# hendraet/synthesis-in-style

Hardware: AMD Instinct MI355X
Metric: StyleGAN2 synth images/sec + seg-train images/sec @256², 1/2/4/8 MI355X (higher is better)
Workload: dtype f32; 1 GPU; StyleGAN2 Generator(256,512,8,cm=2).forward, batch 32 per GPU, explicit noise, return_intermediate_activations=True (BASELINE.json configs[1]); batch_per_gpu=32, image_size=256, parallelism=replicated x1, images sharded, no collective

## Files before the change

### include/sis_hip.h

```cpp
#ifndef SIS_HIP_H
#define SIS_HIP_H

#include <stdint.h>

#ifdef __cplusplus
extern "C" {
#endif

#define SIS_F32 0
#define SIS_F64 1
#define SIS_F16 2
#define SIS_BF16 3

int sis_version(void);
const char* sis_last_error(void);
const char* sis_last_kernel(void);

int sis_fused_bias_act(void* out, const void* x, const void* bias, const void* ref, int dtype,
                       int64_t numel, int64_t step_b, int64_t size_b, int act, int grad,
                       float alpha, float scale, void* stream);

int sis_upfirdn2d_out_size(int in_size, int up, int down, int pad0, int pad1, int k);
int sis_upfirdn2d(void* out, const void* in, const void* taps, int dtype, int major, int in_h,
                  int in_w, int minor, int kh, int kw, int up_x, int up_y, int down_x, int down_y,
                  int pad_x0, int pad_x1, int pad_y0, int pad_y1, void* stream);


int sis_pixel_norm(float* out, const float* x, int batch, int dim, void* stream);

int sis_head_gemm_tile(void);

int sis_equal_linear(float* out, const float* x, int64_t x_row_stride, const float* w,
                     const float* bias, int batch, int in_dim, int out_dim, float scale,
                     float lr_mul, int activation, void* stream);

int sis_modulation_batch(float* out_base, const float* latent, const int64_t* table, int n_layers,
                         int total_blocks, int batch, int n_latent, int dim, float scale, void* stream);

int sis_demod_batch(float* dscale_base, const float* s_base, const int64_t* table, int n_layers,
                    int total_blocks, int batch, void* stream);

int sis_truncate(float* out, const float* w, const float* mean, float psi, int batch, int dim,
                 void* stream);

int sis_modconv_prepack(float* wpk, float* wsq, const float* w, int cout, int cin, int ksize,
                        void* stream);

int sis_modconv_demod(float* dscale, const float* s, const float* wsq, int batch, int cin,
                      int cout, float scale, int demodulate, void* stream);

int sis_modconv2d(float* out, const float* x, const float* wpk, const float* s,
                  const float* dscale, const float* noise, int64_t noise_batch_stride,
                  const float* noise_weight, const float* bias, int batch, int cin, int cout,
                  int h, int w, int ksize, int fuse_act, const float* wino_u, void* workspace,
                  int64_t workspace_bytes, void* stream);

int sis_modconv_prepack_wino(float* u, const float* w, int cout, int cin, void* stream);

int sis_modconv2d_up(float* t, const float* x, const float* wpk, const float* s,
                     const float* dscale, int batch, int cin, int cout, int h, int w,
                     int t_row_stride, void* workspace, int64_t workspace_bytes, void* stream);

int sis_modconv_up_fir_supported(int batch, int cin, int cout, int h, int w, int t_row_stride);
int sis_modconv_up_fir_prepack(float* u, const float* w, int cout, int cin, void* stream);
int sis_modconv2d_up_fir(float* t, const float* x, const float* u, const float* s, const float* dscale, int batch, int cin, int cout,
                         int h, int w, int t_row_stride, void* stream);

int sis_blur_noise_act(float* out, const float* in, const float* taps, const float* noise,
                       int64_t noise_batch_stride, const float* noise_weight, const float* bias,
                       int batch, int channels, int in_h, int in_w, int in_row_stride, int kh, int kw,
                       int pad0, int pad1, int fuse_act, void* stream);

int sis_to_rgb(float* out, const float* x, const float* w, const float* s, const float* bias,
               const float* skip, const float* taps, int batch, int cin, int cout, int h, int width,
               int kh, int kw, int pad0, int pad1, float scale, void* stream);


int sis_upsample_ce_workspace(int batch, int out_h, int out_w);
int sis_upsample_ce_fwd(float* loss, float* workspace, const float* logits, const int64_t* labels,
                        int batch, int classes, int h, int w, int out_h, int out_w,
                        int64_t ignore_index, void* stream);
int sis_upsample_ce_bwd(float* grad_logits, const float* grad_loss, const float* logits,
                        const int64_t* labels, int batch, int classes, int h, int w, int out_h,
                        int out_w, int64_t ignore_index, void* stream);

int sis_sgd_chunk_elems(void);
int sis_sgd_momentum(const int64_t* table, int n_chunks, const float* lr, const float* weight_decay,
                     int n_groups, float momentum, int first_step, void* stream);

int sis_sgd_momentum_dev(const int64_t* table, int n_chunks, const float* hyper, void* stream);

int sis_ema_update(float* mu, const float* mu_batch, float momentum, float one_minus_momentum,
                   int batch, int numel, void* stream);

int sis_half_dilation_taps(float* taps, const float* weight, int cout, int cin, void* stream);
int sis_half_dilation_taps_bwd(float* dweight, const float* dtaps, int cout, int cin, void* stream);

int sis_emau_supported(int batch, int channels, int pixels, int bases);
int64_t sis_emau_workspace_floats(int batch, int channels, int pixels, int bases);
int sis_emau_forward(float* x_out, float* mu_out, const float* x, const float* mu0, float* workspace, int batch, int channels,
                     int pixels, int bases, int stages, void* stream);

int64_t sis_bn_workspace_floats(int batch, int channels, int hw);
int64_t sis_bn_mask_words(int batch, int channels, int hw);
int sis_bn_stats(float* mean, float* invstd, float* running_mean, float* running_var, const float* x,
                 float* workspace, int batch, int channels, int hw, float eps, float momentum, void* stream);
int sis_bn_act_fwd(float* y, const float* x, const float* residual, const float* mean, const float* invstd,
                   const float* gamma, const float* beta, int batch, int channels, int hw, int relu, void* relu_mask,
                   void* stream);
int sis_bn_act_bwd(float* dx, float* dresidual, float* dgamma, float* dbeta, const float* dy, const float* y,
// ... 237 lines not shown
```

### synthesis-in-style_amd/csrc/modconv_wino.hip

```cpp
#include "modconv_common.h"

#if !defined(SIS_ABLATIONS) && (defined(SIS_WINO_NODMA) || defined(SIS_WINO_NOTRANSFORM) || defined(SIS_WINO_NOBARRIER) || \
                                defined(SIS_WINO_NOSTORE) || defined(SIS_WINO_STAGGER))
#error "SIS_WINO_* ablation switches need -DSIS_ABLATIONS (development builds only)"
#endif

namespace {

constexpr int WCC = 8;
#ifndef SIS_WINO_BAR_SLOT
#define SIS_WINO_BAR_SLOT 27
#endif
constexpr int S_BAR = SIS_WINO_BAR_SLOT;
constexpr int WMBLK = 64;
constexpr int WTILES = 64;

__device__ __forceinline__ sis_f32x4 lds_ld4(const float* p) { return *reinterpret_cast<const sis_f32x4*>(p); }
__device__ __forceinline__ void lds_st4(float* p, sis_f32x2 a, sis_f32x2 b) { *reinterpret_cast<sis_f32x4*>(p) = sis_f32x4{a.x, a.y, b.x, b.y}; }
__device__ __forceinline__ float2 lds_ld2(const float* p) {
    const sis_f32x2 d = *reinterpret_cast<const sis_f32x2*>(p);
    return make_float2(d.x, d.y);
}
constexpr unsigned BUF_OOB = 0x80000000u;
__device__ __forceinline__ sis_f32x2 pk_lo_np_plus(sis_f32x2 y, sis_f32x2 np, sis_f32x2 x) {
// ... 834 lines not shown
        const int64_t out_bytes = (int64_t)p.B * p.Cout * p.OH * p.ORS * 4;
        if ((int64_t)want * out_bytes > workspace_bytes) want = (int)(workspace_bytes / out_bytes);
        if (want >= 2) {
            p.kchunk = sis_cdiv(sis_cdiv(p.Cin, want), WCC) * WCC;
            p.ksplit = sis_cdiv(p.Cin, p.kchunk);
            p.slab = (float*)workspace;
        }
    }
    const size_t lds = (size_t)(2 * WCC * 16 * WMBLK + 2 * WCC * tc.xt + (p.s ? p.nb_max * p.Cin : 0)) * sizeof(float);
    const size_t lds2 = lds + (size_t)(2 * 16 * WCC * WTILES + p.nb_max * WMBLK + WMBLK + WTILES * 4) * sizeof(float);
    if (lds > 160 * 1024) return -1;
    if (plan_only) return 0;
    static bool attr_set = false;
    if (!attr_set) {
        hipError_t e = hipFuncSetAttribute(reinterpret_cast<const void*>(&modconv_wino_kernel),
                                           hipFuncAttributeMaxDynamicSharedMemorySize, 160 * 1024);
        if (e != hipSuccess) return sis_fail("modconv: cannot raise the dynamic LDS limit: %s", hipGetErrorString(e));
        attr_set = true;
    }
    static const bool pipelined = !(getenv("SIS_WINO_PIPE") && getenv("SIS_WINO_PIPE")[0] == '0');
    if (pipelined && lds2 <= 160 * 1024 && tc.xt >= 256) {
        sis_kernel_name = "modconv_wino2_kernel";
        static const int tpw_cap = getenv("SIS_WINO_TPW") ? atoi(getenv("SIS_WINO_TPW")) : 16;
        int tpw = 1;
        static const int min_wg = getenv("SIS_WINO_MINWG") ? atoi(getenv("SIS_WINO_MINWG")) : 1024;
        while (p.kchunk % (2 * WCC) == 0 && tpw * 2 <= tpw_cap && p.npos_tiles % (tpw * 2) == 0 && blocks / (tpw * 2) >= min_wg) tpw *= 2;
        static const double swz_mb = getenv("SIS_WINO_XCD_MB") ? atof(getenv("SIS_WINO_XCD_MB")) : 5.0;
        const int64_t grid = blocks / tpw;
        const int n_co_h = (p.Cout + WMBLK - 1) / WMBLK;
        const int xcd_group = (double)p.Cin * p.Cout * 16 * sizeof(float) <= swz_mb * 1048576.0 && n_co_h > 1 && grid % (8 * n_co_h) == 0;
        typedef void (*kern_t)(const ConvParams, const int, const int, const int);
        static const kern_t table[4][2] = {{modconv_wino2_kernel<1, false>, modconv_wino2_kernel<1, true>},
                                           {modconv_wino2_kernel<2, false>, modconv_wino2_kernel<2, true>},
                                           {modconv_wino2_kernel<4, false>, modconv_wino2_kernel<4, true>},
                                           {modconv_wino2_kernel<8, false>, modconv_wino2_kernel<8, true>}};
        static bool table_attr[4][2] = {};
        const int xi_log2 = tc.xt <= 256 ? 0 : tc.xt <= 512 ? 1 : tc.xt <= 1024 ? 2 : 3;
        const kern_t kern = table[xi_log2][p.s ? 1 : 0];
        bool& have_attr = table_attr[xi_log2][p.s ? 1 : 0];
        if (!have_attr) {
            const hipError_t e = hipFuncSetAttribute(reinterpret_cast<const void*>(kern), hipFuncAttributeMaxDynamicSharedMemorySize, 160 * 1024);
            if (e != hipSuccess) return sis_fail("modconv: cannot raise the dynamic LDS limit: %s", hipGetErrorString(e));
            have_attr = true;
        }
        hipLaunchKernelGGL(kern, dim3((unsigned)grid, p.ksplit), dim3(WNTHR), lds2, st, p, tc.xt, tpw, xcd_group);
    } else {
        sis_kernel_name = "modconv_wino_kernel";
        hipLaunchKernelGGL(modconv_wino_kernel, dim3((unsigned)blocks, p.ksplit), dim3(WNTHR), lds, st, p, tc.xt);
    }
    SIS_CHECK_LAUNCH("modconv_wino_kernel");
    if (p.ksplit > 1) modconv_splitk_finish_launch(p, st);
    return 0;
}
```

### synthesis-in-style_amd/networks/stylegan2/model.py

```python
import math
import os
import random
import struct
import typing

import torch
from torch import nn
from torch.nn import functional as F

import sis_hip
from networks import hip_conv
from .op import FusedLeakyReLU, fused_leaky_relu, upfirdn2d

_NOISE_ONE_LAUNCH = os.environ.get('SIS_NOISE_ONE_LAUNCH', '1') != '0'
_RGB_STREAMS = {}


def _needs_grad(*tensors):
    return torch.is_grad_enabled() and any(t is not None and t.requires_grad for t in tensors)


def make_kernel(k):
    taps = torch.tensor(k, dtype=torch.float32)
    if taps.ndim == 1:
# ... 47 lines not shown
    def forward(self, input):
        if _needs_grad(input, self.weight, self.bias) or input.dim() != 2:
            bias = None if self.bias is None else self.bias * self.lr_mul
            if self.activation:
                return fused_leaky_relu(F.linear(input, self.weight * self.scale), bias)
            return F.linear(input, self.weight * self.scale, bias=bias)
        if input.is_contiguous():
            return sis_hip.equal_linear(input, self.weight, self.bias, self.scale, self.lr_mul, self.activation)
        if input.stride(1) != 1:
            input = input.contiguous()
            return sis_hip.equal_linear(input, self.weight, self.bias, self.scale, self.lr_mul, self.activation)
        return sis_hip.equal_linear(input, self.weight, self.bias, self.scale, self.lr_mul, self.activation,
                                    row_stride=input.stride(0), batch=input.shape[0])

    def __repr__(self):
        return f'{self.__class__.__name__}({self.weight.shape[1]}, {self.weight.shape[0]})'


class ModulatedConv2d(nn.Module):
    def __init__(self, in_channel, out_channel, kernel_size, style_dim, demodulate=True, upsample=False,
                 downsample=False, blur_kernel=[1, 3, 3, 1]):
        super().__init__()
        self.eps = 1e-8
        self.kernel_size = kernel_size
        self.in_channel = in_channel
        self.out_channel = out_channel
        self.upsample = upsample
        self.downsample = downsample
        self.demodulate = demodulate
        if upsample:
            factor = 2
            p = (len(blur_kernel) - factor) - (kernel_size - 1)
            self.blur = Blur(blur_kernel, pad=((p + 1) // 2 + factor - 1, p // 2 + 1), upsample_factor=factor)
        if downsample:
            factor = 2
            p = (len(blur_kernel) - factor) + (kernel_size - 1)
            self.blur = Blur(blur_kernel, pad=((p + 1) // 2, p // 2))
        self.scale = 1 / math.sqrt(in_channel * kernel_size ** 2)
        self.padding = kernel_size // 2
        self.weight = nn.Parameter(torch.randn(1, out_channel, in_channel, kernel_size, kernel_size))
        self.modulation = EqualLinear(style_dim, in_channel, bias_init=1)
        self._pack = None
        self._pack_key = None

    def __repr__(self):
        return (f'{self.__class__.__name__}({self.in_channel}, {self.out_channel}, {self.kernel_size}, '
                f'upsample={self.upsample}, downsample={self.downsample})')

    def packed_weights(self):
        w = self.weight
        key = (w.data_ptr(), w._version, w.device)
        if self._pack_key != key:
            self._pack = sis_hip.modconv_prepack(w.detach())
            self._wino = None
            if (self.kernel_size == 3 and not self.upsample and not self.downsample and self.in_channel % 8 == 0
                    and self.out_channel % 4 == 0 and os.environ.get("SIS_WINOGRAD", "1") != "0"):
                self._wino = sis_hip.modconv_prepack_wino(w.detach())
            self._fir = None
            if self.kernel_size == 3 and self.upsample and self.in_channel % 8 == 0 and self.out_channel % 64 == 0:
                self._fir = sis_hip.modconv_prepack_up_fir(w.detach())
            self._pack_key = key
        return self._pack

    def wino_weights(self):
        self.packed_weights()
        return self._wino

    def fir_weights(self):
        self.packed_weights()
        return self._fir

    def hip_supported(self):
        return (not self.downsample) and (self.kernel_size == 3 or (self.kernel_size == 1 and not self.upsample))

    def modulate(self, style):
        wpk, wsq = self.packed_weights()
        s = self.modulation(style)
        return wpk, s, sis_hip.modconv_demod(s, wsq, self.scale, self.demodulate)

    def forward(self, input, style):
        if _needs_grad(input, style, self.weight, self.modulation.weight) or not self.hip_supported():
            return self._forward_autograd(input, style)
        sis_hip.require_device(input, "input")
        wpk, s, dscale = self.modulate(style)
        if self.upsample:
            return self.blur(sis_hip.modconv2d_up(input, wpk, s, dscale))
        return sis_hip.modconv2d(input, wpk, s, dscale, self.kernel_size, wino_u=self.wino_weights())

    def _forward_autograd(self, input, style):
        if self.downsample or os.environ.get("SIS_MODCONV_GROUPED", "0") == "1":
            return self._forward_grouped(input, style)
        b, cin, h, w = input.shape
        k, cout = self.kernel_size, self.out_channel
        s = self.modulation(style)
        weight = self.weight[0]
        if self.demodulate:
            wsq = weight.pow(2).sum((2, 3))
            dcoef = self.scale * torch.rsqrt((self.scale * self.scale) * (s.pow(2) @ wsq.t()) + 1e-8)
        x = input * s.view(b, cin, 1, 1)
        if self.upsample:
            out = F.conv_transpose2d(x, weight.transpose(0, 1), stride=2)
        elif (k == 3 and x.is_cuda and x.is_contiguous() and hip_conv.gan_winograd_enabled()
              and sis_hip.conv3x3_supported(x, weight)):
            out = hip_conv.conv3x3(x, weight)
        else:
            out = F.conv2d(x, weight, padding=self.padding)
        out = out * dcoef.view(b, cout, 1, 1) if self.demodulate else out * self.scale
        return self.blur(out) if self.upsample else out

    def _forward_grouped(self, input, style):
        b, cin, h, w = input.shape
        k, cout = self.kernel_size, self.out_channel
        mod = self.modulation(style).view(b, 1, cin, 1, 1)
        wt = self.scale * self.weight * mod
        if self.demodulate:
            wt = wt * torch.rsqrt(wt.pow(2).sum([2, 3, 4], keepdim=True) + 1e-8)
        x = input.reshape(1, b * cin, h, w)
        if self.upsample:
            out = F.conv_transpose2d(x, wt.transpose(1, 2).reshape(b * cin, cout, k, k), stride=2, groups=b)
            return self.blur(out.view(b, cout, out.shape[2], out.shape[3]))
        if self.downsample:
            x = self.blur(input)
            x = x.reshape(1, b * cin, x.shape[2], x.shape[3])
            out = F.conv2d(x, wt.view(b * cout, cin, k, k), stride=2, groups=b)
        else:
            out = F.conv2d(x, wt.view(b * cout, cin, k, k), padding=self.padding, groups=b)
        return out.view(b, cout, out.shape[2], out.shape[3])


class NoiseInjection(nn.Module):
    def __init__(self):
        super().__init__()
        self.weight = nn.Parameter(torch.zeros(1))

    @staticmethod
    def fresh(image):
        b, _, h, w = image.shape
        return image.new_empty(b, 1, h, w).normal_()

    def forward(self, image, noise=None):
        if noise is None:
            noise = self.fresh(image)
        return image + self.weight * noise


class ConstantInput(nn.Module):
    def __init__(self, channel, size=4):
        super().__init__()
        self.input = nn.Parameter(torch.randn(1, channel, size, size))

    def forward(self, input):
        return self.input.repeat(input.shape[0], 1, 1, 1)


class StyledConv(nn.Module):
    def __init__(self, in_channel, out_channel, kernel_size, style_dim, upsample=False, blur_kernel=[1, 3, 3, 1],
                 demodulate=True):
        super().__init__()
        self.conv = ModulatedConv2d(in_channel, out_channel, kernel_size, style_dim, upsample=upsample,
                                    blur_kernel=blur_kernel, demodulate=demodulate)
        self.noise = NoiseInjection()
        self.activate = FusedLeakyReLU(out_channel)

    def forward(self, input, style, noise=None):
        conv, act = self.conv, self.activate
        fused_ok = (conv.hip_supported() and act.negative_slope == 0.2 and abs(act.scale - 2 ** 0.5) < 1e-12
                    and not _needs_grad(input, style, conv.weight, conv.modulation.weight, self.noise.weight, act.bias))
        if not fused_ok:
            return act(self.noise(conv(input, style), noise=noise))
        sis_hip.require_device(input, "input")
        wpk, s, dscale = conv.modulate(style)
        return self.forward_s(input, wpk, s, dscale, noise)

    def forward_s(self, input, wpk, s, dscale, noise=None, out=None):
        conv, act = self.conv, self.activate
        b, _, h, w = input.shape
        if conv.upsample:
            taps, pad = conv.blur.kernel, conv.blur.pad
            padded = tuple(taps.shape) == (4, 4) and pad[0] == 1
            t = sis_hip.modconv2d_up(input, wpk, s, dscale, padded_rows=padded, fir_u=conv.fir_weights())
            in_w = 2 * w + 1
            oh = t.shape[2] + pad[0] + pad[1] - taps.shape[0] + 1
            ow = in_w + pad[0] + pad[1] - taps.shape[1] + 1
            if noise is None:
                noise = input.new_empty(b, 1, oh, ow).normal_()
            return sis_hip.blur_noise_act(t, taps, pad, noise, self.noise.weight, act.bias, fuse_act=True, in_w=in_w)
        if noise is None:
            noise = input.new_empty(b, 1, h, w).normal_()
        return sis_hip.modconv2d(input, wpk, s, dscale, conv.kernel_size, noise, self.noise.weight, act.bias,
                                 fuse_act=True, wino_u=conv.wino_weights(), out=out)


class ToRGB(nn.Module):
    def __init__(self, in_channel, style_dim, upsample=True, blur_kernel=[1, 3, 3, 1]):
        super().__init__()
        if upsample:
            self.upsample = Upsample(blur_kernel)
        self.conv = ModulatedConv2d(in_channel, 3, 1, style_dim, demodulate=False)
        self.bias = nn.Parameter(torch.zeros(1, 3, 1, 1))

    def forward(self, input, style, skip=None):
        conv = self.conv
        if _needs_grad(input, style, skip, conv.weight, conv.modulation.weight, self.bias):
            out = conv(input, style) + self.bias
            return out if skip is None else out + self.upsample(skip)
        sis_hip.require_device(input, "input")
        return self.forward_s(input, conv.modulation(style), skip)

    def forward_s(self, input, s, skip=None, out=None):
        conv = self.conv
        if skip is None:
            return sis_hip.to_rgb(input, conv.weight, s, self.bias, conv.scale, out=out)
        up = self.upsample
        if up.factor != 2:
            return sis_hip.to_rgb(input, conv.weight, s, self.bias, conv.scale) + up(skip)
        return sis_hip.to_rgb(input, conv.weight, s, self.bias, conv.scale, skip, up.kernel, up.pad, out=out)


def truncate_styles(style, truncation, truncation_latent):
    if _needs_grad(style, truncation_latent) or not style.is_cuda or truncation_latent.numel() != style.shape[-1]:
        return truncation_latent + truncation * (style - truncation_latent)
    return sis_hip.truncate(style, truncation_latent, truncation)


def resolve_latents(generator, styles, inject_index, truncation, truncation_latent, input_is_latent, noise,
                    randomize_noise):
    if not input_is_latent:
        styles = [generator.style(s) for s in styles]
    if noise is None:
        noise = [None] * generator.num_layers if randomize_noise else [
            getattr(generator.noises, f'noise_{i}') for i in range(generator.num_layers)]
    if truncation < 1:
        styles = [truncate_styles(s, truncation, truncation_latent) for s in styles]
    n_latent = generator.n_latent
    if len(styles) < 2:
        latent = styles[0].unsqueeze(1).repeat(1, n_latent, 1) if styles[0].ndim < 3 else styles[0]
    else:
        if inject_index is None:
            inject_index = random.randint(1, n_latent - 1)
        latent = torch.cat([styles[0].unsqueeze(1).repeat(1, inject_index, 1),
                            styles[1].unsqueeze(1).repeat(1, n_latent - inject_index, 1)], 1)
    return latent, noise

# ... 232 lines not shown
```

### synthesis-in-style_amd/sis_hip/__init__.py

```python
import collections
import ctypes
import os

import torch

_HERE = os.path.dirname(os.path.abspath(__file__))
LIB_PATH = os.path.join(os.path.dirname(_HERE), "lib", os.environ.get("SIS_HIP_LIB", "libsis_hip.so"))

_lib = None

F32, F64, F16, BF16 = 0, 1, 2, 3
_DTYPE_CODE = {torch.float32: F32, torch.float64: F64, torch.float16: F16, torch.bfloat16: BF16}

_vp, _i, _i64, _f = ctypes.c_void_p, ctypes.c_int, ctypes.c_int64, ctypes.c_float
_d = ctypes.c_double

_SIGNATURES = {
    "sis_version": ([], _i),
    "sis_last_error": ([], ctypes.c_char_p),
    "sis_fused_bias_act": ([_vp, _vp, _vp, _vp, _i, _i64, _i64, _i64, _i, _i, _f, _f, _vp], _i),
    "sis_upfirdn2d_out_size": ([_i] * 6, _i),
    "sis_upfirdn2d": ([_vp, _vp, _vp] + [_i] * 15 + [_vp], _i),
    "sis_pixel_norm": ([_vp, _vp, _i, _i, _vp], _i),
    "sis_equal_linear": ([_vp, _vp, _i64, _vp, _vp, _i, _i, _i, _f, _f, _i, _vp], _i),
    "sis_truncate": ([_vp, _vp, _vp, _f, _i, _i, _vp], _i),
    "sis_modulation_batch": ([_vp, _vp, _vp, _i, _i, _i, _i, _i, _f, _vp], _i),
    "sis_demod_batch": ([_vp, _vp, _vp, _i, _i, _i, _vp], _i),
    "sis_modconv_prepack": ([_vp, _vp, _vp, _i, _i, _i, _vp], _i),
    "sis_modconv_demod": ([_vp, _vp, _vp, _i, _i, _i, _f, _i, _vp], _i),
    "sis_modconv2d": ([_vp, _vp, _vp, _vp, _vp, _vp, _i64, _vp, _vp] + [_i] * 7 + [_vp, _vp, _i64, _vp], _i),
    "sis_head_gemm_tile": ([], _i),
    "sis_modconv_prepack_wino": ([_vp, _vp, _i, _i, _vp], _i),
    "sis_last_kernel": ([], ctypes.c_char_p),
    "sis_conv3x3_prepack": ([_vp, _vp, _i, _i, _i, _vp], _i),
    "sis_conv3x3_prepack_both": ([_vp, _vp, _vp, _i, _i, _vp], _i),
    "sis_conv3x3_prepack_multi": ([_vp, _i, _i, _vp], _i),
    "sis_conv3x3_eligible": ([_i] * 5, _i),
    "sis_upsample_bilinear": ([_vp, _vp, _i, _i64, _i, _i, _i, _i, _i, _vp], _i),
    "sis_upsample_bilinear_strided": ([_vp, _vp, _i, _i, _i, _i, _i, _i, _i, _i64, _i, _vp], _i),
    "sis_gemm_bf16_workspace_bytes": ([_i, _i, _i], _i64),
    "sis_gemm_bf16": ([_vp] * 4 + [_i] * 8 + [_vp] * 3 + [_i] + [_vp] * 3 + [_i, _f, _i, _vp, _i64, _i, _vp], _i),
    "sis_gemm_bf16_wgrad_bias": ([_vp] * 4 + [_i] * 6 + [_vp, _i64, _i, _vp], _i),
    "sis_gemm_bf16_wgrad_multi_workspace_bytes": ([_i, _i, _i], _i64),
    "sis_gemm_bf16_wgrad_bias_multi": ([_vp] * 4 + [_i] * 6 + [_vp, _i64, _i, _vp], _i),
    "sis_gemm_bf16_batched": ([_vp] * 3 + [_i] * 9 + [_i64] * 3 + [_i, _vp, _i64, _i, _vp], _i),
    "sis_layer_norm_bwd_fused": ([_vp] * 9 + [_i, _i, _i, _i, _vp, _vp, _vp, _i, _f, _vp], _i),
    "sis_attention_fwd": ([_vp, _vp, _vp, _i, _i, _i, _vp], _i),
    "sis_attention_bwd": ([_vp] * 6 + [_i, _i, _i, _vp], _i),
    "sis_ce_dice_workspace_floats": ([_i], _i),
    "sis_ce_dice_fwd": ([_vp] * 4 + [_i, _vp, _i, _i, _i, _vp], _i),
    "sis_ce_dice_bwd": ([_vp, _vp, _i, _vp, _vp, _vp, _i, _i, _i, _vp], _i),
    "sis_dropout_advance": ([_vp, _vp], _i),
    "sis_dropout_bwd_cast": ([_vp, _vp, _i64, _vp, _i, _f, _vp], _i),
    "sis_layer_norm_workspace_floats": ([_i], _i),
    "sis_layer_norm_bwd_fused_partial": ([_vp] * 7 + [_i, _i, _i, _i, _vp, _vp, _vp, _i, _f, _vp], _i),
    "sis_layer_norm_bwd_parts": ([_i], _i),
    "sis_layer_norm_param_reduce_multi": ([_vp] * 5 + [_i, _vp], _i),
    "sis_column_sum_workspace_floats": ([_i], _i64),
    "sis_column_sum": ([_vp, _vp, _vp, _i, _i, _i, _vp], _i),
    "sis_layer_norm_fwd": ([_vp] * 6 + [_i, _i, _i, _i, _f, _vp], _i),
    "sis_layer_norm_bwd": ([_vp] * 9 + [_i, _i, _i, _i, _vp], _i),
    "sis_weight_std_fwd": ([_vp, _vp, _vp, _i, _i, _i, _f, _vp], _i),
    "sis_group_norm_fwd": ([_vp] * 9 + [_i, _i, _i, _i, _i, _i, _f, _i, _vp, _vp, _vp], _i),
    "sis_group_norm_gate_bytes": ([_i, _i, _i], _i64),
    "sis_group_norm_workspace_floats": ([_i, _i, _i], _i64),
    "sis_batch_norm_fwd": ([_vp] * 9 + [_i] * 5 + [_f, _f, _i, _vp, _vp], _i),
    "sis_batch_norm_bwd": ([_vp] * 10 + [_i] * 6 + [_vp, _vp], _i),
    "sis_group_norm_bwd": ([_vp] * 13 + [_i] * 7 + [_vp, _vp, _vp], _i),
    "sis_weight_std_bwd": ([_vp, _vp, _vp, _vp, _i, _i, _i, _f, _vp], _i),
    "sis_conv3x3_wgrad_eligible": ([_i] * 5 + [_i64], _i),
    "sis_conv3x3_wgrad": ([_vp, _vp, _vp, _i, _i, _i, _i, _i, _vp, _i64, _vp], _i),
    "sis_conv3x3_wgrad_multi": ([_vp, _vp, _vp, _i, _i, _i, _i, _i, _i, _vp, _i64, _vp], _i),
    "sis_conv3x3": ([_vp, _vp, _vp, _i, _i, _i, _i, _i, _vp, _i64, _vp], _i),
    "sis_modconv2d_up": ([_vp] * 5 + [_i] * 6 + [_vp, _i64, _vp], _i),
    "sis_modconv_up_fir_supported": ([_i] * 6, _i),
    "sis_modconv_up_fir_prepack": ([_vp, _vp, _i, _i, _vp], _i),
    "sis_modconv2d_up_fir": ([_vp] * 5 + [_i] * 6 + [_vp], _i),
    "sis_blur_noise_act": ([_vp, _vp, _vp, _vp, _i64, _vp, _vp] + [_i] * 10 + [_vp], _i),
    "sis_to_rgb": ([_vp] * 7 + [_i] * 9 + [_f, _vp], _i),
    "sis_conv1x1_wgrad_f32_supported": ([_i] * 4, _i),
    "sis_conv1x1_wgrad_f32_workspace": ([_i] * 4, _i64),
    "sis_conv1x1_wgrad_f32": ([_vp, _vp, _vp, _i, _i, _i, _i, _vp, _i64, _vp], _i),
    "sis_conv1x1_wgrad_f32_multi": ([_vp, _vp, _vp, _i, _i, _i, _i, _i, _vp, _i64, _vp], _i),
    "sis_max_pool2d": ([_vp, _vp, _vp, _i, _i64] + [_i] * 8 + [_vp], _i),
    "sis_upsample_ce_workspace": ([_i] * 3, _i),
# ... 326 lines not shown

def head_gemm_tile():
    return int(lib().sis_head_gemm_tile())


def modulation_batch(out_flat, latent, table, n_layers, total_blocks, scale):
    b, n_latent, dim = latent.shape
    with torch.cuda.device(latent.device):
        _check(lib().sis_modulation_batch(_ptr(out_flat), _ptr(latent), _ptr(table), n_layers, total_blocks, b, n_latent,
                                          dim, float(scale), _stream()), "sis_modulation_batch")


def demod_batch(dscale_flat, s_flat, table, n_layers, total_blocks, batch):
    with torch.cuda.device(s_flat.device):
        _check(lib().sis_demod_batch(_ptr(dscale_flat), _ptr(s_flat), _ptr(table), n_layers, total_blocks, batch,
                                     _stream()), "sis_demod_batch")


def truncate(w, mean, psi):
    w = _f32(w, "style")
    mean = _f32(mean, "truncation_latent").reshape(-1)
    dim = w.shape[-1]
    if mean.numel() != dim:
        raise RuntimeError("truncation_latent must hold one latent vector")
    out = torch.empty_like(w)
    with torch.cuda.device(w.device):
        _check(lib().sis_truncate(_ptr(out), _ptr(w), _ptr(mean), float(psi), w.numel() // dim, dim, _stream()),
               "sis_truncate")
    return out


def modconv_prepack(weight):
    w = _f32(weight, "weight")
    _, cout, cin, k, _ = w.shape
    wpk = torch.empty((cin, k * k, cout), dtype=torch.float32, device=w.device)
    wsq = torch.empty((cout, cin), dtype=torch.float32, device=w.device)
    with torch.cuda.device(w.device):
        _check(lib().sis_modconv_prepack(_ptr(wpk), _ptr(wsq), _ptr(w), cout, cin, k, _stream()),
               "sis_modconv_prepack")
    return wpk, wsq


def modconv_prepack_wino(weight):
    w = _f32(weight, "weight")
    _, cout, cin, k, _ = w.shape
    if k != 3:
        raise RuntimeError("the Winograd transform is for 3x3 kernels")
    u = torch.empty((cin, 16, cout), dtype=torch.float32, device=w.device)
    with torch.cuda.device(w.device):
        _check(lib().sis_modconv_prepack_wino(_ptr(u), _ptr(w), cout, cin, _stream()), "sis_modconv_prepack_wino")
    return u


def conv3x3_supported(x, weight, dilation=1):
    if not (x.is_cuda and x.dtype == torch.float32 and x.dim() == 4 and weight.dim() == 4
            and tuple(weight.shape[2:]) == (3, 3) and weight.shape[1] == x.shape[1]):
        return False
    b, _, h, w = x.shape
    d = int(dilation)
    if d < 1 or h % d or w % d:
        return False
    cout, cin = weight.shape[0], weight.shape[1]
    if cout % 8 or cin % 8:
        return False
    key = (b * d * d, cin, cout, h // d, w // d)
    hit = _conv3x3_ok.get(key)
    if hit is None:
        hit = bool(lib().sis_conv3x3_eligible(*key)) and bool(lib().sis_conv3x3_eligible(key[0], cout, cin, key[3], key[4]))
        _conv3x3_ok[key] = hit
    return hit


_conv3x3_ok = {}


def conv3x3_prepack(weight, adjoint=False):
    w = _f32(weight, "weight")
    cout_w, cin_w = w.shape[0], w.shape[1]
    cout, cin = (cin_w, cout_w) if adjoint else (cout_w, cin_w)
    u = torch.empty((cin, 16, cout), dtype=torch.float32, device=w.device)
    with torch.cuda.device(w.device):
        _check(lib().sis_conv3x3_prepack(_ptr(u), _ptr(w), cout, cin, int(bool(adjoint)), _stream()), "sis_conv3x3_prepack")
    return u


def conv3x3_prepack_both(weight):
    w = _f32(weight, "weight")
    cout, cin = w.shape[0], w.shape[1]
    u = torch.empty((cin, 16, cout), dtype=torch.float32, device=w.device)
    ua = torch.empty((cout, 16, cin), dtype=torch.float32, device=w.device)
    with torch.cuda.device(w.device):
        _check(lib().sis_conv3x3_prepack_both(_ptr(u), _ptr(ua), _ptr(w), cout, cin, _stream()), "sis_conv3x3_prepack_both")
    return u, ua


class WinogradPackBank:

    def __init__(self, weights):
        self.weights = [w for w in weights]
        dev = self.weights[0].device
        self.u, self.u_adjoint, rows, block = [], [], [], 0
        for w in self.weights:
            if w.dtype != torch.float32 or not w.is_contiguous() or w.dim() != 4 or tuple(w.shape[2:]) != (3, 3):
                raise RuntimeError("WinogradPackBank: contiguous float32 [Cout, Cin, 3, 3] weights only")
            cout, cin = w.shape[0], w.shape[1]
            self.u.append(torch.empty((cin, 16, cout), dtype=torch.float32, device=dev))
# ... 229 lines not shown
    _deferred["wgrad"].setdefault(key, []).append((grad.data_ptr(), x.data_ptr(), dw.data_ptr(), db.data_ptr(), _hold(grad, x, dw, db)))
    return dw, db


def flush_deferred():
    if _deferred["conv"]:
        _flush_conv_wgrads()
    if _deferred["wgrad"]:
        queued, _deferred["wgrad"] = _deferred["wgrad"], {}
        for key, jobs in queued.items():
            _wgrad_multi_raw([j[:4] for j in jobs], key)
    jobs = _deferred["ln"]
    if jobs:
        _deferred["ln"] = []
        n = len(jobs)
        vp, ci = ctypes.c_void_p * n, ctypes.c_int * n
        with torch.cuda.device(jobs[0][5]):
            _check(lib().sis_layer_norm_param_reduce_multi(vp(*[j[0] for j in jobs]), vp(*[j[1] for j in jobs]), vp(*[j[2] for j in jobs]),
                                                           ci(*[j[3] for j in jobs]), ci(*[j[4] for j in jobs]), n, _stream()),
                   "sis_layer_norm_param_reduce_multi")


WORKSPACE_BYTES = int(os.environ.get("SIS_WORKSPACE_MB", "128")) << 20
_workspaces = {}


def _workspace(device):
    ws = _workspaces.get(device)
    if ws is None:
        ws = torch.empty(WORKSPACE_BYTES, dtype=torch.uint8, device=device)
        _workspaces[device] = ws
    return ws


def _noise_args(noise, batch, h, w):
    if noise is None:
        return None, 0
    noise = _f32(noise, "noise")
    if noise.numel() == h * w:
        return noise, 0
    if noise.numel() == batch * h * w:
        return noise, h * w
    raise RuntimeError(f"noise shape {tuple(noise.shape)} does not broadcast over [{batch}, C, {h}, {w}]")


def _out_or_new(out, shape, device, what):
    if out is None:
        return torch.empty(shape, dtype=torch.float32, device=device)
    if tuple(out.shape) != tuple(shape) or out.dtype != torch.float32 or not out.is_contiguous() or out.device != device:
        raise RuntimeError(f"{what}: out must be a contiguous float32 tensor of shape {tuple(shape)} on {device}")
    return out


def modconv2d(x, wpk, s, dscale, ksize, noise=None, noise_weight=None, bias=None, fuse_act=False, wino_u=None, out=None):
    x = _f32(x, "input")
    batch, cin, h, w = x.shape
    cout = wpk.shape[2]
    noise, nbs = _noise_args(noise, batch, h, w)
    out = _out_or_new(out, (batch, cout, h, w), x.device, "modconv2d")
    ws = _workspace(x.device)
    wino = wino_u is not None and ksize == 3 and h % 2 == 0 and w % 2 == 0 and cin % 8 == 0 and cout % 4 == 0
    with torch.cuda.device(x.device):
        _check(_launch(None,
                       2.0 * batch * cout * cin * ksize * ksize * h * w,
                       4.0 * (x.numel() + out.numel() + wpk.numel()),
                       lambda: lib().sis_modconv2d(_ptr(out), _ptr(x), _ptr(wpk), _ptr(s), _ptr(dscale), _ptr(noise),
                                                   nbs, _ptr(noise_weight), _ptr(bias), batch, cin, cout, h, w, ksize,
                                                   int(bool(fuse_act)), _ptr(wino_u), _ptr(ws), ws.numel(), _stream())),
               "sis_modconv2d")
    return out


_UP_FIR = os.environ.get("SIS_UP_FIR", "1") != "0"


def modconv_prepack_up_fir(weight):
    w = _f32(weight, "weight")
    if w.dim() == 5:
        w = w[0]
    cout, cin = w.shape[0], w.shape[1]
    u = torch.empty((cin, 8, cout, 2), dtype=torch.float32, device=w.device)
    with torch.cuda.device(w.device):
        _check(lib().sis_modconv_up_fir_prepack(_ptr(u), _ptr(w), cout, cin, _stream()), "sis_modconv_up_fir_prepack")
    return u


def modconv2d_up(x, wpk, s, dscale, padded_rows=False, fir_u=None):
    x = _f32(x, "input")
    batch, cin, h, w = x.shape
    cout = wpk.shape[2]
    row = 2 * w + 4 if padded_rows else 2 * w + 1
    out = torch.empty((batch, cout, 2 * h + 1, row), dtype=torch.float32, device=x.device)
    if fir_u is not None and _UP_FIR and padded_rows and lib().sis_modconv_up_fir_supported(batch, cin, cout, h, w, row):
        with torch.cuda.device(x.device):
            _check(_launch(None, 2.0 * batch * cout * cin * 9 * h * w, 4.0 * (x.numel() + out.numel() + fir_u.numel()),
                           lambda: lib().sis_modconv2d_up_fir(_ptr(out), _ptr(x), _ptr(fir_u), _ptr(s), _ptr(dscale), batch, cin, cout,
                                                              h, w, row, _stream())), "sis_modconv2d_up_fir")
        return out
    ws = _workspace(x.device)
    with torch.cuda.device(x.device):
        _check(_launch(None, 2.0 * batch * cout * cin * 9 * h * w,
                       4.0 * (x.numel() + out.numel() + wpk.numel()),
                       lambda: lib().sis_modconv2d_up(_ptr(out), _ptr(x), _ptr(wpk), _ptr(s), _ptr(dscale), batch, cin,
                                                      cout, h, w, row, _ptr(ws), ws.numel(), _stream())),
               "sis_modconv2d_up")
    return out


def blur_noise_act(x, taps, pad, noise=None, noise_weight=None, bias=None, fuse_act=False, in_w=None):
    x = _f32(x, "input")
    taps = _f32(taps, "kernel")
    batch, ch, ih, row_stride = x.shape
# ... 1635 lines not shown
```

Measured before the change: 2274 images/s.

## Add Winograd F(2x4,3x3) modulated conv kernel and route eligible layers to it

Adds a new Winograd variant that uses 2x4 output tiles (a 4x6 input transform, 24 products) for 3x3 modulated convolutions. It comes with its own weight prepack, an eligibility check and a fused noise/bias/leaky-ReLU epilogue. Layers that qualify now use it instead of the existing F(2x2) Winograd path. The aim is fewer multiplies per output and less transform overhead per tile, at the cost of larger LDS use, heavier transforms, more f32 rounding error and a lot of new hand-scheduled kernel code.

```diff
diff --git a/include/sis_hip.h b/include/sis_hip.h
--- a/include/sis_hip.h
+++ b/include/sis_hip.h
@@ -56,6 +56,12 @@
                   int64_t workspace_bytes, void* stream);
 
 int sis_modconv_prepack_wino(float* u, const float* w, int cout, int cin, void* stream);
+
+int sis_modconv_prepack_wino24(float* u, const float* w, int cout, int cin, void* stream);
+int sis_modconv_wino24_eligible(int cin, int cout, int h, int w);
+int sis_modconv2d_wino24(float* out, const float* x, const float* u24, const float* s, const float* dscale,
+                         const float* noise, int64_t noise_batch_stride, const float* noise_weight, const float* bias,
+                         int batch, int cin, int cout, int h, int w, int fuse_act, int tiles_per_wg, void* stream);
 
 int sis_modconv2d_up(float* t, const float* x, const float* wpk, const float* s,
                      const float* dscale, int batch, int cin, int cout, int h, int w,
diff --git a/synthesis-in-style_amd/csrc/modconv_wino.hip b/synthesis-in-style_amd/csrc/modconv_wino.hip
--- a/synthesis-in-style_amd/csrc/modconv_wino.hip
+++ b/synthesis-in-style_amd/csrc/modconv_wino.hip
@@ -910,3 +910,5 @@
     if (p.ksplit > 1) modconv_splitk_finish_launch(p, st);
     return 0;
 }
+
+#include "modconv_wino24.h"
diff --git a/synthesis-in-style_amd/csrc/modconv_wino24.h b/synthesis-in-style_amd/csrc/modconv_wino24.h
--- /dev/null
+++ b/synthesis-in-style_amd/csrc/modconv_wino24.h
@@ -0,0 +1,373 @@
+
+namespace {
+
+constexpr int W24_CC = 4;
+constexpr int W24_UF = W24_CC * 24 * WMBLK;
+constexpr int W24_VF = W24_CC * 24 * WTILES;
+constexpr int W24_XT = 720;
+constexpr int W24_XP = 3;
+constexpr int W24_BAR = 19;
+
+__global__ __launch_bounds__(256) void wino24_prepack_kernel(float* __restrict__ u, const float* __restrict__ w, int cout, int cin) {
+    const int64_t idx = (int64_t)blockIdx.x * 256 + threadIdx.x;
+    if (idx >= (int64_t)cout * cin) return;
+    const int co = (int)(idx % cout), ci = (int)(idx / cout);
+    const float* g = w + ((int64_t)co * cin + ci) * 9;
+    float t[4][3];
+#pragma unroll
+    for (int c = 0; c < 3; ++c) {
+        const float g0 = g[c], g1 = g[3 + c], g2 = g[6 + c];
+        t[0][c] = g0;
+        t[1][c] = 0.5f * (g0 + g1 + g2);
+        t[2][c] = 0.5f * (g0 - g1 + g2);
+        t[3][c] = g2;
+    }
+#pragma unroll
+    for (int i = 0; i < 4; ++i) {
+        const float a = t[i][0], b = t[i][1], c = t[i][2];
+        const float o[6] = {0.25f * a,
+                            (-1.f / 6.f) * (a + b + c),
+                            (-1.f / 6.f) * (a - b + c),
+                            (1.f / 24.f) * a + (1.f / 12.f) * b + (1.f / 6.f) * c,
+                            (1.f / 24.f) * a - (1.f / 12.f) * b + (1.f / 6.f) * c,
+                            c};
+#pragma unroll
+        for (int j = 0; j < 6; ++j) {
+            const int q = j / 3, e = 3 * i + j % 3;
+            u[((((int64_t)ci * 2 + q) * 3 + (e >> 2)) * cout + co) * 4 + (e & 3)] = o[j];
+        }
+    }
+}
+
+__global__ __launch_bounds__(WNTHR, 2) void modconv_wino24_kernel(const ConvParams p, const int tiles_per_wg, const int xcd_group) {
+    constexpr int CC = W24_CC, UF = W24_UF, VF = W24_VF, XT = W24_XT;
+    extern __shared__ __attribute__((aligned(16))) float lds[];
+    float* Ul = lds;
+    float* Vl = Ul + 2 * UF;
+    float* Xl = Vl + 2 * VF;
+    float* Sl = Xl + 2 * CC * XT;
+    float* Dl = Sl + p.Cin;
+    float* Bl = Dl + WMBLK;
+    float* Nl = Bl + WMBLK;
+
+    const int tid = threadIdx.x, lane = tid & 63, wave = __builtin_amdgcn_readfirstlane(tid >> 6);
+    const int l31 = lane & 31, half = lane >> 5;
+    const int q = wave & 1, wn = (wave >> 1) & 1, wm = wave >> 2;
+
+    const int n_co = p.Cout / WMBLK;
+    const int wg = xcd_group ? (int)(blockIdx.x & 7) * (int)(gridDim.x >> 3) + (int)(blockIdx.x >> 3) : (int)blockIdx.x;
+    const int o0 = (wg % n_co) * WMBLK;
+    const TileClass tc = p.cls[0];
+    const int thl = tc.th_log2, twl = tc.tw_log2;
+    const int tw = 1 << twl;
+    const int ew = tw + 8, ew4 = ew >> 2;
+    const int HW = p.H * p.W;
+    const int k_hi = p.Cin, k_last = k_hi - CC;
+
+    const __amdgpu_buffer_rsrc_t u_rsrc = sis_buffer_rsrc(p.wpk + (int64_t)o0 * 4);
+    const unsigned u_voff = (unsigned)lane * 16u;
+    const unsigned u_row_bytes = (unsigned)p.Cout * 16u;
+    auto stage_u_piece = [&](int ci0, int buf, int it) {
+        sis_buffer_load_lds16(u_rsrc, Ul + buf * UF + (wave + it * 8) * 256, u_voff, (unsigned)(ci0 * 6 + wave + it * 8) * u_row_bytes);
+    };
+    int xp_ch[2], xp_base[2];
+#pragma unroll
+    for (int k = 0; k < 2; ++k) {
+        const int piece = k == 0 ? wave : (wave + 8) % (CC * W24_XP);
+        xp_ch[k] = piece / W24_XP;
+        xp_base[k] = min((piece % W24_XP) * 256, XT - 256);
+    }
+    struct TileState {
+        int b, h0, w0;
+        unsigned xv[2];
+        __amdgpu_buffer_rsrc_t x_rsrc;
+    } T;
+    auto tile_setup = [&](int pt, TileState& S, int lane) {
+        const int twi = pt % tc.ntw; pt /= tc.ntw;
+        const int thi = pt % tc.nth;
+        S.b = pt / tc.nth; S.h0 = thi << thl; S.w0 = twi << twl;
+#pragma unroll
+        for (int k = 0; k < 2; ++k) {
+            const int f4 = (xp_base[k] >> 2) + lane;
+            const int r = f4 / ew4, c4 = f4 - r * ew4;
+            const int h = S.h0 - 1 + r, w = S.w0 - 4 + 4 * c4;
+            S.xv[k] = (h >= 0 && h < p.H && w >= 0 && w < p.W) ? (unsigned)(h * p.W + w) * 4u : BUF_OOB;
+        }
+        S.x_rsrc = sis_buffer_rsrc(p.x + (int64_t)S.b * p.Cin * HW);
+    };
+    auto stage_x_piece = [&](int ci0, int buf, int k) {
+        sis_buffer_load_lds16(T.x_rsrc, Xl + buf * CC * XT + xp_ch[k] * XT + xp_base[k], T.xv[k], (unsigned)((ci0 + xp_ch[k]) * HW) * 4u);
+    };
+    const int pt_first = wg / n_co, pt_step = gridDim.x / n_co;
+    const int txs = twl - 2;
+    const float noise_w0 = (p.fuse && p.noise) ? p.noise_w[0] : 0.f;
+
+    auto run = [&](auto qc) {
+        constexpr int Q = decltype(qc)::value;
+        const int tch = wave >> 1;
+        const int txo = tch * XT + 2 * (lane >> txs) * ew + 4 * (lane & ((1 << txs) - 1));
+        constexpr int teo = Q == 0 ? 3 : 8;
+        const int tvo = (tch * 2 + Q) * 3 * (WTILES * 4) + lane * 4;
+        float sv = 1.f, de[4], ee[4][3], oo[4][3];
+        sis_f32x4 dm[4];
+        auto t_read = [&](const float* xb, int r) {
+            dm[r] = lds_ld4(xb + r * ew + 4);
+            de[r] = xb[r * ew + teo];
+        };
+        auto t_col = [&](int r) {
+            const float a = dm[r].x, b = dm[r].y, c = dm[r].z, d = dm[r].w, e = de[r];
+            if (Q == 0) {
+                const float u = fmaf(-4.f, b, d), v = fmaf(-4.f, a, c);
+                ee[r][0] = fmaf(4.f, e, fmaf(-5.f, b, d));
+                ee[r][1] = u + v;
+                ee[r][2] = u - v;
+            } else {
+                const float u = d - b, v = c - a;
+                ee[r][0] = fmaf(2.f, v, u);
+                ee[r][1] = fmaf(-2.f, v, u);
+                ee[r][2] = fmaf(4.f, a, fmaf(-5.f, c, e));
+            }
+        };
+        auto t_row = [&](int jj) {
+            oo[0][jj] = (ee[0][jj] - ee[2][jj]) * sv;
+            oo[1][jj] = (ee[1][jj] + ee[2][jj]) * sv;
+            oo[2][jj] = (ee[2][jj] - ee[1][jj]) * sv;
+            oo[3][jj] = (ee[1][jj] - ee[3][jj]) * sv;
+        };
+        auto t_write = [&](float* vw) {
+            *reinterpret_cast<sis_f32x4*>(vw) = sis_f32x4{oo[0][0], oo[0][1], oo[0][2], oo[1][0]};
+            *reinterpret_cast<sis_f32x4*>(vw + WTILES * 4) = sis_f32x4{oo[1][1], oo[1][2], oo[2][0], oo[2][1]};
+            *reinterpret_cast<sis_f32x4*>(vw + 2 * WTILES * 4) = sis_f32x4{oo[2][2], oo[3][0], oo[3][1], oo[3][2]};
+        };
+        const int aoff = (half * 2 + Q) * 3 * (WMBLK * 4) + (wm * 32 + l31) * 4;
+        const int voff = (half * 2 + Q) * 3 * (WTILES * 4) + (wn * 32 + l31) * 4;
+
+        sis_f32x16 acc[12];
+        sis_f32x4 ou[2], ov[2];
+
+        for (int k = 0; k < tiles_per_wg; ++k) {
+#pragma unroll
+            for (int e = 0; e < 12; ++e)
+#pragma unroll
+                for (int j = 0; j < 16; ++j) acc[e][j] = 0.f;
+            int tp = tid;
+            asm volatile("" : "+v"(tp));
+            tile_setup(pt_first + k * pt_step, T, tp & 63);
+            if (k > 0) __syncthreads();
+#pragma unroll
+            for (int it = 0; it < 3; ++it) stage_u_piece(0, 0, it);
+#pragma unroll
+            for (int kx = 0; kx < 2; ++kx) stage_x_piece(0, 0, kx);
+#pragma unroll
+            for (int kx = 0; kx < 2; ++kx) stage_x_piece(min(CC, k_last), 1, kx);
+            for (int e = tp; e < p.Cin; e += WNTHR) Sl[e] = p.s[(int64_t)T.b * p.Cin + e];
+            if (tp < WMBLK) {
+                Dl[tp] = p.dscale[(int64_t)T.b * p.Cout + o0 + tp];
+                Bl[tp] = (p.fuse && p.bias) ? p.bias[o0 + tp] : 0.f;
+            }
+            {
+                const int tt_ = tp >> 3, e = tp & 7;
+                const int yy = T.h0 + 2 * (tt_ >> txs) + (e >> 2), xx = T.w0 + 4 * (tt_ & ((1 << txs) - 1)) + (e & 3);
+                float nv = 0.f;
+                if (p.fuse && p.noise && yy < p.H && xx < p.W) nv = noise_w0 * p.noise[(int64_t)T.b * p.noise_bstride + yy * p.W + xx];
+                Nl[tp] = nv;
+            }
+            asm volatile("s_waitcnt vmcnt(0)" ::: "memory");
+            __syncthreads();
+            sv = Sl[tch];
+#pragma unroll
+            for (int r = 0; r < 4; ++r) t_read(Xl + txo, r);
+#pragma unroll
+            for (int r = 0; r < 4; ++r) t_col(r);
+#pragma unroll
+            for (int jj = 0; jj < 3; ++jj) t_row(jj);
+            t_write(Vl + tvo);
+            __syncthreads();
+            ou[0] = lds_ld4(Ul + aoff);
+            ov[0] = lds_ld4(Vl + voff);
+
+            auto chunk = [&](auto parity, const int ci0) {
+                constexpr int cur = decltype(parity)::value, nxt = cur ^ 1;
+                const int uci = ci0 + CC >= k_hi ? 0 : ci0 + CC;
+                const int xci = min(ci0 + 2 * CC, k_last);
+                const int tci = min(ci0 + CC, k_last);
+                const float* Ub = Ul + cur * UF + aoff;
+                const float* Vb = Vl + cur * VF + voff;
+                const float* xb = Xl + nxt * CC * XT + txo;
+                float* vw = Vl + nxt * VF + tvo;
+#pragma unroll
+                for (int sl = 0; sl < 24; ++sl) {
+                    const int g = sl >> 2, part = sl & 3, slot = g & 1;
+                    const int e = (g % 3) * 4 + part;
+                    const float ua = part == 0 ? ou[slot].x : part == 1 ? ou[slot].y : part == 2 ? ou[slot].z : ou[slot].w;
+                    const float va = part == 0 ? ov[slot].x : part == 1 ? ov[slot].y : part == 2 ? ov[slot].z : ov[slot].w;
+                    acc[e] = __builtin_amdgcn_mfma_f32_32x32x2f32(ua, va, acc[e], 0, 0, 0);
+                    if (part == 0 && g < 5) {
+                        ou[slot ^ 1] = lds_ld4(Ub + (12 * ((g + 1) / 3) + (g + 1) % 3) * WMBLK * 4);
+                        ov[slot ^ 1] = lds_ld4(Vb + (12 * ((g + 1) / 3) + (g + 1) % 3) * WTILES * 4);
+                    }
+                    if (sl == 2 || sl == 6 || sl == 10) stage_u_piece(uci, nxt, (sl - 2) >> 2);
+                    if (sl == 13) stage_x_piece(xci, cur, 0);
+                    if (sl == 15) stage_x_piece(xci, cur, 1);
+                    if (sl == 1) { sv = Sl[tci + tch]; t_read(xb, 0); t_read(xb, 1); }
+                    if (sl == 3) t_read(xb, 2);
+                    if (sl == 5) { t_read(xb, 3); t_col(0); }
+                    if (sl == 7) t_col(1);
+                    if (sl == 9) t_col(2);
+                    if (sl == 11) t_col(3);
+                    if (sl == 12) t_row(0);
+                    if (sl == 14) t_row(1);
+                    if (sl == 16) t_row(2);
+                    if (sl == 17) t_write(vw);
+                    if (sl == W24_BAR) {
+                        asm volatile("s_waitcnt vmcnt(0)" ::: "memory");
+                        __syncthreads();
+                    }
+                    if (sl == 23) {
+                        ou[0] = lds_ld4(Ul + nxt * UF + aoff);
+                        ov[0] = lds_ld4(Vl + nxt * VF + voff);
+                    }
+                    __builtin_amdgcn_sched_barrier(0);
+                }
+            };
+            for (int ci0 = 0; ci0 < k_hi; ci0 += 2 * CC) {
+                chunk(std::integral_constant<int, 0>(), ci0);
+                chunk(std::integral_constant<int, 1>(), ci0 + CC);
+            }
+
+            float mine[8][2][3];
+            int te = tid;
+            asm volatile("" : "+v"(te));
+            const int lane = te & 63, l31 = te & 31, half = (te >> 5) & 1;
+            float* xch = lds + (wave >> 1) * (2 * 48 * 64);
+#pragma unroll
+            for (int jo = 0; jo < 16; ++jo) {
+                const int j = (jo + 8 * (1 - Q)) & 15;
+#pragma unroll
+                for (int jj = 0; jj < 3; ++jj) {
+                    const float a0 = acc[jj][j], a1 = acc[3 + jj][j], a2 = acc[6 + jj][j], a3 = acc[9 + jj][j];
+                    const float m0 = a0 + a1 + a2, m1 = a1 - a2 - a3;
+                    if ((j >> 3) == Q) {
+                        mine[j & 7][0][jj] = m0;
+                        mine[j & 7][1][jj] = m1;
+                    } else {
+                        xch[(Q * 48 + (j & 7) * 6 + jj) * 64 + lane] = m0;
+                        xch[(Q * 48 + (j & 7) * 6 + 3 + jj) * 64 + lane] = m1;
+                    }
+                }
+            }
+            __syncthreads();
+
+            const int t = wn * 32 + l31;
+            const int oh = T.h0 + 2 * (t >> txs), ow = T.w0 + 4 * (t & ((1 << txs) - 1));
+            if (oh < p.H && ow < p.W) {
+                const float slope = p.fuse ? 0.2f : 1.f, gain = p.fuse ? 1.4142135623730951f : 1.f;
+                const int cl0 = wm * 32 + 16 * Q + 4 * half;
+                float* obase = p.out + ((int64_t)T.b * p.Cout + o0 + cl0) * HW + oh * p.W + ow;
+                const float* xin = xch + (1 - Q) * 48 * 64 + lane;
+                const sis_f32x4 nz0 = lds_ld4(Nl + t * 8), nz1 = lds_ld4(Nl + t * 8 + 4);
+#pragma unroll
+                for (int jr = 0; jr < 8; ++jr) {
+                    const int ro = (jr & 3) + 8 * (jr >> 2);
+                    const float dd = Dl[cl0 + ro], bb = Bl[cl0 + ro];
+                    float theirs[2][3];
+#pragma unroll
+                    for (int e = 0; e < 6; ++e) theirs[e / 3][e % 3] = xin[(jr * 6 + e) * 64];
+#pragma unroll
+                    for (int r = 0; r < 2; ++r) {
+                        const float* ma = Q == 0 ? mine[jr][r] : theirs[r];
+                        const float* mb = Q == 0 ? theirs[r] : mine[jr][r];
+                        const float sa = ma[1] + ma[2], da = ma[1] - ma[2], sb = mb[0] + mb[1], db = mb[0] - mb[1];
+                        const float y[4] = {(ma[0] + sa) + sb, fmaf(2.f, db, da), fmaf(4.f, sb, sa), fmaf(8.f, db, da) + mb[2]};
+                        const sis_f32x4 nz = r == 0 ? nz0 : nz1;
+                        const float nzv[4] = {nz.x, nz.y, nz.z, nz.w};
+                        float o[4];
+#pragma unroll
+                        for (int x = 0; x < 4; ++x) {
+                            float val = y[x] * dd;
+                            val += nzv[x];
+                            val += bb;
+                            o[x] = fmaxf(val, val * slope) * gain;
+                        }
+                        *reinterpret_cast<sis_f32x4*>(obase + (int64_t)ro * HW + r * p.W) = sis_f32x4{o[0], o[1], o[2], o[3]};
+                    }
+                }
+            }
+        }
+    };
+    if (q == 0) run(std::integral_constant<int, 0>());
+    else run(std::integral_constant<int, 1>());
+}
+
+}
+
+extern "C" int sis_modconv_prepack_wino24(float* u, const float* w, int cout, int cin, void* stream) {
+    SIS_REQUIRE(u && w, "sis_modconv_prepack_wino24: null pointer");
+    SIS_REQUIRE(cout > 0 && cin > 0, "sis_modconv_prepack_wino24: bad sizes");
+    hipLaunchKernelGGL(wino24_prepack_kernel, dim3(sis_cdiv((int64_t)cout * cin, 256)), dim3(256), 0, (hipStream_t)stream, u, w, cout, cin);
+    SIS_CHECK_LAUNCH("sis_modconv_prepack_wino24");
+    return 0;
+}
+
+static int wino24_plan(ConvParams& p, int cin, int cout, int h, int w) {
+    if (cin <= 0 || cout <= 0 || h <= 0 || w <= 0) return -1;
+    if (cin % 8 || cout % WMBLK || h % 2 || w % 4) return -1;
+    if ((int64_t)cin * h * w * 4 >= ((int64_t)1 << 31) || (int64_t)cin * cout * 96 >= ((int64_t)1 << 31)) return -1;
+    p.slab = nullptr; p.ksplit = 1; p.kchunk = cin; p.npos_tiles = 0; p.ncls = 0; p.nb_max = 0;
+    mc_add_class(p, 512, 2, 1, 0, h, 0, w, 64, 1);
+    const TileClass& tc = p.cls[0];
+    if (tc.nb != 1 || tc.th_log2 + tc.tw_log2 != 9 || tc.tw_log2 < 5) return -1;
+    if (((1 << tc.th_log2) + 2) * ((1 << tc.tw_log2) + 8) != W24_XT) return -1;
+    const size_t lds = (size_t)(2 * W24_UF + 2 * W24_VF + 2 * W24_CC * W24_XT + cin + 2 * WMBLK + WTILES * 8) * sizeof(float);
+    if (lds > 160 * 1024) return -1;
+    return (int)lds;
+}
+
+extern "C" int sis_modconv_wino24_eligible(int cin, int cout, int h, int w) {
+    ConvParams p;
+    return wino24_plan(p, cin, cout, h, w) > 0 ? 1 : 0;
+}
+
+extern "C" int sis_modconv2d_wino24(float* out, const float* x, const float* u24, const float* s, const float* dscale,
+                                    const float* noise, int64_t noise_batch_stride, const float* noise_weight, const float* bias,
+                                    int batch, int cin, int cout, int h, int w, int fuse_act, int tiles_per_wg, void* stream) {
+    if (batch == 0) return 0;
+    SIS_REQUIRE(out && x && u24 && s && dscale, "sis_modconv2d_wino24: null pointer");
+    SIS_REQUIRE(batch > 0, "sis_modconv2d_wino24: non-positive size");
+    if (noise) SIS_REQUIRE(noise_weight, "sis_modconv2d_wino24: noise given without noise_weight");
+    ConvParams p;
+    const int lds = wino24_plan(p, cin, cout, h, w);
+    SIS_REQUIRE(lds > 0, "sis_modconv2d_wino24: shape %dx%d, %d -> %d not eligible (sis_modconv_wino24_eligible)", h, w, cin, cout);
+    SIS_REQUIRE((int64_t)batch * (cin > cout ? cin : cout) * h * w < ((int64_t)1 << 31), "sis_modconv2d_wino24: tensor too large");
+    SIS_REQUIRE(((((uintptr_t)x | (uintptr_t)u24 | (uintptr_t)out) & 15) == 0) && (!noise || ((uintptr_t)noise & 3) == 0),
+                "sis_modconv2d_wino24: pointers must be 16-byte aligned");
+    p.x = x; p.wpk = u24; p.s = s; p.dscale = dscale; p.noise = noise; p.noise_w = noise_weight; p.bias = bias;
+    p.out = out; p.noise_bstride = noise_batch_stride;
+    p.B = batch; p.Cin = cin; p.Cout = cout; p.H = h; p.W = w; p.OH = h; p.OW = w; p.ORS = w; p.fuse = fuse_act != 0;
+    p.cout_vec4 = 1;
+    const TileClass& tc = p.cls[0];
+    const int64_t tiles = (int64_t)batch * tc.nth * tc.ntw;
+    p.npos_tiles = (int)tiles;
+    const int n_co = cout / WMBLK;
+    const int64_t blocks = tiles * n_co;
+    SIS_REQUIRE(blocks < ((int64_t)1 << 31), "sis_modconv2d_wino24: bad grid");
+    int tpw = 1;
+    if (tiles_per_wg > 0) {
+        SIS_REQUIRE(tiles % tiles_per_wg == 0, "sis_modconv2d_wino24: %d tiles per workgroup do not divide %lld tiles", tiles_per_wg, (long long)tiles);
+        tpw = tiles_per_wg;
+    } else {
+        while (tpw * 2 <= 16 && tiles % (tpw * 2) == 0 && blocks / (tpw * 2) >= 1024) tpw *= 2;
+    }
+    const int64_t grid = blocks / tpw;
+    const int xcd_group = (double)cin * cout * 24 * sizeof(float) <= 5.0 * 1048576.0 && n_co > 1 && grid % (8 * n_co) == 0;
+    static bool have_attr = false;
+    if (!have_attr) {
+        const hipError_t e = hipFuncSetAttribute(reinterpret_cast<const void*>(&modconv_wino24_kernel), hipFuncAttributeMaxDynamicSharedMemorySize, 160 * 1024);
+        if (e != hipSuccess) return sis_fail("modconv: cannot raise the dynamic LDS limit: %s", hipGetErrorString(e));
+        have_attr = true;
+    }
+    sis_kernel_name = "modconv_wino24_kernel";
+    hipLaunchKernelGGL(modconv_wino24_kernel, dim3((unsigned)grid), dim3(WNTHR), (size_t)lds, (hipStream_t)stream, p, tpw, xcd_group);
+    SIS_CHECK_LAUNCH("modconv_wino24_kernel");
+    return 0;
+}
diff --git a/synthesis-in-style_amd/networks/stylegan2/model.py b/synthesis-in-style_amd/networks/stylegan2/model.py
--- a/synthesis-in-style_amd/networks/stylegan2/model.py
+++ b/synthesis-in-style_amd/networks/stylegan2/model.py
@@ -123,10 +123,10 @@
         key = (w.data_ptr(), w._version, w.device)
         if self._pack_key != key:
             self._pack = sis_hip.modconv_prepack(w.detach())
-            self._wino = None
-            if (self.kernel_size == 3 and not self.upsample and not self.downsample and self.in_channel % 8 == 0
-                    and self.out_channel % 4 == 0 and os.environ.get("SIS_WINOGRAD", "1") != "0"):
-                self._wino = sis_hip.modconv_prepack_wino(w.detach())
+            self._wino = self._wino24 = None
+            self._wino_on = (self.kernel_size == 3 and not self.upsample and not self.downsample and self.in_channel % 8 == 0
+                             and self.out_channel % 4 == 0 and os.environ.get("SIS_WINOGRAD", "1") != "0")
+            self._wino24_on = self._wino_on and os.environ.get("SIS_WINO24", "1") != "0"
             self._fir = None
             if self.kernel_size == 3 and self.upsample and self.in_channel % 8 == 0 and self.out_channel % 64 == 0:
                 self._fir = sis_hip.modconv_prepack_up_fir(w.detach())
@@ -135,7 +135,17 @@
 
     def wino_weights(self):
         self.packed_weights()
+        if self._wino is None and self._wino_on:
+            self._wino = sis_hip.modconv_prepack_wino(self.weight.detach())
         return self._wino
+
+    def winograd_operand(self, h, w):
+        self.packed_weights()
+        if self._wino24_on and sis_hip.modconv_wino24_eligible(self.in_channel, self.out_channel, h, w):
+            if self._wino24 is None:
+                self._wino24 = sis_hip.modconv_prepack_wino24(self.weight.detach())
+            return {"wino24_u": self._wino24}
+        return {"wino_u": self.wino_weights()}
 
     def fir_weights(self):
         self.packed_weights()
@@ -156,7 +166,7 @@
         wpk, s, dscale = self.modulate(style)
         if self.upsample:
             return self.blur(sis_hip.modconv2d_up(input, wpk, s, dscale))
-        return sis_hip.modconv2d(input, wpk, s, dscale, self.kernel_size, wino_u=self.wino_weights())
+        return sis_hip.modconv2d(input, wpk, s, dscale, self.kernel_size, **self.winograd_operand(*input.shape[2:]))
 
     def _forward_autograd(self, input, style):
         if self.downsample or os.environ.get("SIS_MODCONV_GROUPED", "0") == "1":
@@ -259,7 +269,7 @@
         if noise is None:
             noise = input.new_empty(b, 1, h, w).normal_()
         return sis_hip.modconv2d(input, wpk, s, dscale, conv.kernel_size, noise, self.noise.weight, act.bias,
-                                 fuse_act=True, wino_u=conv.wino_weights(), out=out)
+                                 fuse_act=True, out=out, **conv.winograd_operand(h, w))
 
 
 class ToRGB(nn.Module):
diff --git a/synthesis-in-style_amd/sis_hip/__init__.py b/synthesis-in-style_amd/sis_hip/__init__.py
--- a/synthesis-in-style_amd/sis_hip/__init__.py
+++ b/synthesis-in-style_amd/sis_hip/__init__.py
@@ -31,6 +31,9 @@
     "sis_modconv2d": ([_vp, _vp, _vp, _vp, _vp, _vp, _i64, _vp, _vp] + [_i] * 7 + [_vp, _vp, _i64, _vp], _i),
     "sis_head_gemm_tile": ([], _i),
     "sis_modconv_prepack_wino": ([_vp, _vp, _i, _i, _vp], _i),
+    "sis_modconv_prepack_wino24": ([_vp, _vp, _i, _i, _vp], _i),
+    "sis_modconv_wino24_eligible": ([_i] * 4, _i),
+    "sis_modconv2d_wino24": ([_vp] * 6 + [_i64, _vp, _vp] + [_i] * 7 + [_vp], _i),
     "sis_last_kernel": ([], ctypes.c_char_p),
     "sis_conv3x3_prepack": ([_vp, _vp, _i, _i, _i, _vp], _i),
     "sis_conv3x3_prepack_both": ([_vp, _vp, _vp, _i, _i, _vp], _i),
@@ -463,6 +466,21 @@
     return u
 
 
+def modconv_prepack_wino24(weight):
+    w = _f32(weight, "weight")
+    _, cout, cin, k, _ = w.shape
+    if k != 3:
+        raise RuntimeError("the Winograd transform is for 3x3 kernels")
+    u = torch.empty((cin, 2, 3, cout, 4), dtype=torch.float32, device=w.device)
+    with torch.cuda.device(w.device):
+        _check(lib().sis_modconv_prepack_wino24(_ptr(u), _ptr(w), cout, cin, _stream()), "sis_modconv_prepack_wino24")
+    return u
+
+
+def modconv_wino24_eligible(cin, cout, h, w):
+    return bool(lib().sis_modconv_wino24_eligible(int(cin), int(cout), int(h), int(w)))
+
+
 def conv3x3_supported(x, weight, dilation=1):
     if not (x.is_cuda and x.dtype == torch.float32 and x.dim() == 4 and weight.dim() == 4
             and tuple(weight.shape[2:]) == (3, 3) and weight.shape[1] == x.shape[1]):
@@ -798,12 +816,23 @@
     return out
 
 
-def modconv2d(x, wpk, s, dscale, ksize, noise=None, noise_weight=None, bias=None, fuse_act=False, wino_u=None, out=None):
+def modconv2d(x, wpk, s, dscale, ksize, noise=None, noise_weight=None, bias=None, fuse_act=False, wino_u=None, out=None,
+              wino24_u=None, wino24_tiles_per_wg=0):
     x = _f32(x, "input")
     batch, cin, h, w = x.shape
     cout = wpk.shape[2]
     noise, nbs = _noise_args(noise, batch, h, w)
     out = _out_or_new(out, (batch, cout, h, w), x.device, "modconv2d")
+    if wino24_u is not None and ksize == 3 and batch > 0 and modconv_wino24_eligible(cin, cout, h, w):
+        with torch.cuda.device(x.device):
+            _check(_launch(None,
+                           0.75 * 2.0 * batch * cout * cin * 9 * h * w,
+                           4.0 * (x.numel() + out.numel() + wino24_u.numel()),
+                           lambda: lib().sis_modconv2d_wino24(_ptr(out), _ptr(x), _ptr(wino24_u), _ptr(s), _ptr(dscale), _ptr(noise),
+                                                              nbs, _ptr(noise_weight), _ptr(bias), batch, cin, cout, h, w,
+                                                              int(bool(fuse_act)), int(wino24_tiles_per_wg), _stream())),
+                   "sis_modconv2d_wino24")
+        return out
     ws = _workspace(x.device)
     wino = wino_u is not None and ksize == 3 and h % 2 == 0 and w % 2 == 0 and cin % 8 == 0 and cout % 4 == 0
     with torch.cuda.device(x.device):
```

Measured after the change: 2489 images/s, median of 6. 1.09x the previous value.
